# dune-community/pylrbms

Measured on AMD Instinct MI355X. Metric: offline project+estimate throughput, higher is better.
Workload: dtype f64

## Files before the change

include/lrbms_hip.h:

```cpp
#ifndef LRBMS_HIP_H
#define LRBMS_HIP_H

#include <stdint.h>

#ifdef __cplusplus
extern "C" {
#endif

#define LRBMS_OK 0
#define LRBMS_E_INVALID (-1)
#define LRBMS_E_HIP (-2)
#define LRBMS_E_STATE (-3)
#define LRBMS_E_NOT_CONVERGED (-4)

#define LRBMS_NS 16

typedef struct lrbms_ctx lrbms_ctx;

typedef struct {
  int32_t kx, ky, n_T, n_rt, n_vertices, ncf;
  double hx, hy;
  double kappa[4];
  const int32_t* nb_elem;
  const int32_t* nb_face;
// ... 52 lines not shown
} lrbms_quadrature;
int lrbms_set_quadrature(lrbms_ctx* ctx, const lrbms_quadrature* quad);

int lrbms_assemble_swipdg(lrbms_ctx* ctx, int32_t Q, const double* lam, double* A_diag, double* A_cpl, void* stream);

int lrbms_assemble_rhs(lrbms_ctx* ctx, const double* f_smp, const double* lhat, double* b, double* f2, double* ceps,
                       void* stream);

int lrbms_assemble_products(lrbms_ctx* ctx, int32_t Q, const double* theta_bar, const double* lam, const double* lam_df,
                            const double* lbar, const double* lhat, double* P_diag, double* ebar, double* caa, double* Aab,
                            double* Bbb, void* stream);

int lrbms_assemble_flux(lrbms_ctx* ctx, int32_t Q, const double* lam, double* F, void* stream);

int lrbms_oswald_apply(lrbms_ctx* ctx, int32_t N, const double* V, double* Wt, void* stream);

int lrbms_flux_reconstruct(lrbms_ctx* ctx, int32_t Q, int32_t N, const double* F, const double* V, double* Rt,
                           void* stream);

int lrbms_project_system(lrbms_ctx* ctx, int32_t Q, int32_t N, const double* V, const double* A_diag,
                         const double* A_cpl, const double* P_diag, const double* b, double* work, double* B_sys,
                         double* rhs_red, double* E_red, double* M_red, void* stream);

int64_t lrbms_estimator_work_size(lrbms_ctx* ctx, int32_t Q, int32_t N);
int lrbms_estimator_grams(lrbms_ctx* ctx, int32_t Q, int32_t N, const double* V, const double* Wt, const double* Rt,
                          const double* ebar, const double* caa, const double* Aab, const double* Bbb,
                          const double* b, double* work, double* G_nc, double* r_fd, double* G_rdd, double* G_bb,
                          double* G_ab, double* G_aa, void* stream);

int lrbms_fused_supported(lrbms_ctx* ctx, int32_t Q, int32_t N);
int32_t lrbms_fused_fnc_ld(lrbms_ctx* ctx, int32_t N);
int64_t lrbms_fused_mfma_per_subdomain(lrbms_ctx* ctx, int32_t Q, int32_t N);
int lrbms_fused_factored_supported(lrbms_ctx* ctx, int32_t Q, int32_t N);
int64_t lrbms_fused_work_size(lrbms_ctx* ctx, int32_t Q, int32_t N);
int lrbms_project_estimate_fused(lrbms_ctx* ctx, int32_t Q, int32_t N, const double* V, const double* F,
                                 const double* A_diag, const double* A_cpl, const double* P_diag, const double* b,
                                 const double* ebar, const double* caa, const double* Aab, const double* Bbb,
                                 double* work, double* B_sys, double* rhs_red, double* E_red, double* M_red,
                                 double* G_nc, double* r_fd, double* G_rdd, double* G_bb, double* G_ab, double* G_aa,
                                 void* stream);

void* lrbms_ctx_aux_stream(lrbms_ctx* ctx, int32_t i);

#define LRBMS_OPT_OSWALD_VERTEX_PATCH 9
#define LRBMS_OPT_OSWALD_ZERO_ON_SUBDOMAIN_BOUNDARY 1
#define LRBMS_OPT_ACCUMULATE_COUPLING_ACROSS_Q 2
#define LRBMS_OPT_STREAMS 3
#define LRBMS_OPT_F1_KSPLIT 4
#define LRBMS_OPT_F1_FORM 5
#define LRBMS_OPT_COARSE 6
#define LRBMS_OPT_SOLVE_VALU 7
#define LRBMS_OPT_ESTIMATE_VALU 8
#define LRBMS_OPT_PREP_LDS 10
int lrbms_ctx_set_option(lrbms_ctx* ctx, int32_t option, int32_t value);

int lrbms_set_diagonal_neighbours(lrbms_ctx* ctx, const int32_t* nbr_diag);

int lrbms_fused_set_subset(lrbms_ctx* ctx, const int32_t* subset, int32_t count);

int lrbms_kernel_timing(lrbms_ctx* ctx, int32_t enable);
int lrbms_kernel_timing_read(lrbms_ctx* ctx, char* names, int64_t names_cap, double* ms, int32_t cap, int32_t* count);

int lrbms_project_estimate_fused_phase(lrbms_ctx* ctx, int32_t phase, int32_t Q, int32_t N, const double* V, const double* F,
                                       const double* A_diag, const double* A_cpl, const double* P_diag, const double* b,
                                       const double* ebar, const double* caa, const double* Aab, const double* Bbb, double* work,
                                       double* B_sys, double* rhs_red, double* E_red, double* M_red, double* G_nc, double* r_fd,
                                       double* G_rdd, double* G_bb, double* G_ab, double* G_aa, void* stream);

int64_t lrbms_fside_size(lrbms_ctx* ctx, int32_t Q, int32_t N);
int64_t lrbms_fnc_size(lrbms_ctx* ctx, int32_t N);
int lrbms_project_estimate_fused_factored(lrbms_ctx* ctx, int32_t phase, int32_t Q, int32_t N, const double* V, const double* F,
                                          const double* A_diag, const double* A_cpl, const double* P_diag, const double* b,
                                          const double* ebar, const double* caa, const double* Aab, const double* Bbb, double* work,
                                          double* B_sys, double* rhs_red, double* E_red, double* M_red, double* G_nc_self,
                                          double* r_fd, double* G_rdd_self, double* G_bb_self, double* G_ab_self, double* G_aa,
                                          double* F_side, double* F_nc, void* stream);
int lrbms_reduced_estimate_factored(lrbms_ctx* ctx, int32_t Q, int32_t N, const double* theta, const double* u,
                                    const double* G_nc_self, const double* r_fd, const double* G_rdd_self, const double* G_bb_self,
                                    const double* G_ab_self, const double* G_aa, const double* F_side, const double* F_nc,
                                    const double* f2, const double* ceps, double hdiam, double* eta_loc, void* stream);
int lrbms_reduced_estimate_batch_factored(lrbms_ctx* ctx, int32_t Q, int32_t N, int32_t nmu, const double* theta, const double* u,
                                          const double* G_nc_self, const double* r_fd, const double* G_rdd_self,
                                          const double* G_bb_self, const double* G_ab_self, const double* G_aa, const double* F_side,
                                          const double* F_nc, const double* f2, const double* ceps, double hdiam, double* eta_loc,
                                          void* stream);

int lrbms_reduced_estimate(lrbms_ctx* ctx, int32_t Q, int32_t N, const double* theta, const double* u,
                           const double* G_nc, const double* r_fd, const double* G_rdd, const double* G_bb,
                           const double* G_ab, const double* G_aa, const double* f2, const double* ceps, double hdiam,
                           double* eta_loc, void* stream);

int lrbms_reduced_estimate_batch(lrbms_ctx* ctx, int32_t Q, int32_t N, int32_t nmu, const double* theta, const double* u,
                                 const double* G_nc, const double* r_fd, const double* G_rdd, const double* G_bb,
                                 const double* G_ab, const double* G_aa, const double* f2, const double* ceps, double hdiam,
                                 double* eta_loc, void* stream);

int64_t lrbms_reduced_solve_work_size(lrbms_ctx* ctx, int32_t N);
int lrbms_reduced_solve(lrbms_ctx* ctx, int32_t Q, int32_t N, const double* theta, const double* B_sys,
                        const double* rhs_red, double* work, double* u, double rtol, int32_t max_iter, double* info,
                        void* stream);

int64_t lrbms_reduced_solve_batch_work_size(lrbms_ctx* ctx, int32_t N, int32_t nmu);
int lrbms_reduced_solve_batch(lrbms_ctx* ctx, int32_t Q, int32_t N, int32_t nmu, const double* theta, const double* B_sys,
                              const double* rhs_red, double* work, double* u, double rtol, int32_t max_iter, double* info,
                              void* stream);

// ... 62 lines not shown
```

pylrbms_amd/_isa_check.py:

```python
import re


class IsaCheckError(RuntimeError):
    pass


def _functions(path):
    cur, out = None, {}
    with open(path) as fh:
        for ln in fh:
            m = re.match(r'^(_Z\w+):\s+; @', ln)
            if m:
                cur = m.group(1)
                out[cur] = []
                continue
            if cur is not None:
                if ln.startswith('.Lfunc_end'):
                    cur = None
                    continue
                out[cur].append(ln.rstrip('\n'))
    return out


def _metadata(path):
# ... 101 lines not shown
                break
            if op.startswith('s_cbranch') and toks and toks[-1] in label_at:
                succ.append(label_at[toks[-1]])
                continue
            touched = frozenset().union(*[_regs(t) for t in toks]) if toks else frozenset()
            if touched:
                ev.append(('T', touched, st))
        if fall and nxt[b] < len(lines):
            succ.append(nxt[b])
        blocks[b] = (ev, succ)
    bad, seen = set(), set()
    first = 0 if inside is None else max(b for b in starts if b <= min(inside))
    work = [(first, ())]
    while work:
        b, state = work.pop()
        if inside is not None and b not in inside and b != first:
            continue
        if (b, state) in seen:
            continue
        seen.add((b, state))
        if len(seen) > max_states:
            raise IsaCheckError('in-flight register analysis: more than {} (block, state) pairs'.format(max_states))
        pending = list(state)
        ev, succ = blocks[b]
        live = frozenset().union(*pending) if pending else frozenset()
        settled = False
        for e in ev:
            if e[0] == 'W':
                pending = pending[len(pending) - e[1]:] if e[1] else []
                live = frozenset().union(*pending) if pending else frozenset()
                if prologue_of is not None and not pending and b in prologue_of:
                    settled = True
                    break
            elif e[0] == 'L':
                pending = (pending + [e[1]])[-63:]
                live = live | e[1]
            elif live and e[1] & live:
                bad.add(e[2])
        if settled:
            continue
        out = tuple(pending)
        for t in succ:
            if (t, out) not in seen:
                work.append((t, out))
    return sorted(bad)


def check_fused_isa(asm_path):
    fns = _functions(asm_path)
    meta = _metadata(asm_path)
    report, problems = [], []
    seen = 0
    for name, lines in fns.items():
        m = re.search(r'\dk_f(1u|1v|1|2)I((?:Li\d+E)+)E', name) or re.search(r'\dk_f(1w)()E4Tmpl', name)
        if not m:
            continue
        kernel = 'k_f{}<{}>'.format(m.group(1), ','.join(re.findall(r'Li(\d+)E', m.group(2))))
        md = meta.get(name, {})
        spills = md.get('vgpr_spill_count', 0)
        scratch_lines = [i for i, ln in enumerate(lines) if re.match(r'\s+scratch_', ln)]
        in_asm = False
        first_asm_load = None
        for i, ln in enumerate(lines):
            st = ln.strip()
            if st.startswith(';;#ASMSTART'):
                in_asm = True
            elif st.startswith(';;#ASMEND'):
                in_asm = False
            elif in_asm and 'global_load' in ln:
                first_asm_load = i
                break
        wide = m.group(1) in ('1', '1u') and re.findall(r'Li(\d+)E', m.group(2))[0] == '4'
        if (spills or scratch_lines or md.get('private_segment_fixed_size', 0)) and not wide:
            problems.append('{}: scratch {} bytes, {} spilled VGPRs'.format(kernel, md.get('private_segment_fixed_size'), spills))
        if spills > 8:
            problems.append('{}: {} spilled VGPRs'.format(kernel, spills))
        if scratch_lines and first_asm_load is not None and max(scratch_lines) >= first_asm_load:
            problems.append('{}: scratch instruction behind the first asm-managed load (line {} >= {})'.format(
                kernel, max(scratch_lines), first_asm_load))
        lean = m.group(1) in ('1v', '1w')
        uses_asm_prefetch = any(';;#ASMSTART' in ln for ln in lines) and \
            any('global_load' in ln for ln in lines if True) and \
            any(re.search(r'^\s+s_waitcnt vmcnt\((?!0\))\d+\)\s*$' if not lean else r'^\s+s_waitcnt vmcnt\(0\)\s*$', ln) for ln in lines)
        loops, tags = _producer_loops(lines)
        if m.group(1) == '1' and kernel.endswith(',0>'):
            report.append('{}: compiler-managed loads, VGPRs {}'.format(kernel, md.get('vgpr_count')))
            continue
        if not loops or not uses_asm_prefetch:
            problems.append('{}: no producer loop with asm-managed prefetch found'.format(kernel))
            continue
        seen += 1
        if lean:
            loop_blocks = set()
            starts_all = sorted({0} | {i for i, ln in enumerate(lines) if re.match(r'^\.LBB\d+_\d+:', ln)})
            for idx in loops:
                members = set(idx)
                loop_blocks |= {b for b in starts_all if b in members}
            hz = _inflight_register_hazards(lines, tags, region=None, prologue_of=loop_blocks)
            if hz:
                problems.append('{}: compiler-emitted instruction touches the destination of an asm load of the PROLOGUE still in flight: {}'.format(
                    kernel, hz[:3]))
        for idx in loops:
            hazards = _inflight_register_hazards(lines, tags, region=idx)
            if hazards:
                problems.append('{}: compiler-emitted instruction touches the destination of an asm load still in flight: {}'.format(
                    kernel, hazards[:3]))
            a, b = idx[0], idx[-1]
# ... 45 lines not shown
```

pylrbms_amd/_native.py:

```python
import ctypes
import os

import numpy as np

_HERE = os.path.dirname(os.path.abspath(__file__))
LIB_PATH = os.path.join(_HERE, 'liblrbms_hip.so')

c_i32, c_i64, c_dbl, c_vp = ctypes.c_int32, ctypes.c_int64, ctypes.c_double, ctypes.c_void_p
_P_I32 = ctypes.POINTER(c_i32)
_P_DBL = ctypes.POINTER(c_dbl)


class MeshDesc(ctypes.Structure):
    _fields_ = ([(k, c_i32) for k in ('kx', 'ky', 'n_T', 'n_rt', 'n_vertices', 'ncf')] +
                [('hx', c_dbl), ('hy', c_dbl), ('kappa', c_dbl * 4)] +
                [(k, _P_I32) for k in ('nb_elem', 'nb_face', 'nb_elem_out', 'nb_face_out', 'elem_side_pos', 'elem_rt',
                                       'face_sign', 'dof_vertex', 'vdof_ptr', 'vdof_idx', 'rt_e0', 'rt_f0', 'rt_e1',
                                       'rt_f1', 'rt_side', 'side_elem', 'side_elem_out', 'side_count')] +
                [('ntouch', c_i32), ('touch_elem', _P_I32), ('touch_count', _P_I32)] +
                [(k, _P_DBL) for k in ('grad', 'area', 'normal', 'face_len', 'points')])


SIGNATURES = {
    'lrbms_version': (ctypes.c_char_p, []),
# ... 418 lines not shown
        self._check(rc, 'lrbms_reduced_solve')
        return u, {'iterations': int(info[0]), 'relative_residual': float(info[1])}

    def reduced_solve_batch(self, thetas, B_sys, rhs_red, rtol=1e-13, max_iter=20000, work=None):
        Q, S, N = B_sys.shape[0], self.S, B_sys.shape[3]
        th = np.ascontiguousarray(thetas, dtype=np.float64)
        nmu = th.shape[0]
        assert th.shape == (nmu, Q)
        need = int(self.lib.lrbms_reduced_solve_batch_work_size(self.handle, N, nmu))
        if work is None:
            work = self.empty(need)
        if work.numel() < need:
            raise NativeError('reduced_solve_batch: work too small')
        u = self.empty(S, N, nmu)
        info = np.zeros(2)
        rc = self.lib.lrbms_reduced_solve_batch(self.handle, Q, N, nmu, _dblp(th), self._ptr(B_sys, (Q, S, 5, N, N), 'B_sys'),
                                                self._ptr(rhs_red, (S, N), 'rhs_red'), c_vp(work.data_ptr()),
                                                c_vp(u.data_ptr()), float(rtol), int(max_iter), _dblp(info), self._stream())
        self._check(rc, 'lrbms_reduced_solve_batch')
        return u, {'iterations': int(info[0]), 'relative_residual': float(info[1])}

    def reduced_solve_batches(self, thetas, B_sys, rhs_red, per_call=64, rtol=1e-13, max_iter=20000, concat=True):
        torch = self.torch
        th = np.ascontiguousarray(thetas, dtype=np.float64)
        per_call = max(1, min(int(per_call), 64))
        work = self.empty(int(self.lib.lrbms_reduced_solve_batch_work_size(self.handle, int(B_sys.shape[3]), min(per_call, th.shape[0]))))
        res = [self.reduced_solve_batch(th[b0:b0 + per_call], B_sys, rhs_red, rtol=rtol, max_iter=max_iter, work=work)
               for b0 in range(0, th.shape[0], per_call)]
        if concat:
            u = torch.cat([r[0] for r in res], dim=2) if len(res) > 1 else res[0][0]
        else:
            u = [r[0] for r in res]
        return u, {'iterations': max(r[1]['iterations'] for r in res), 'relative_residual': max(r[1]['relative_residual'] for r in res)}

    def reduced_precond_build(self, theta, B_sys):
        Q, S, N = B_sys.shape[0], self.S, B_sys.shape[3]
        th = np.ascontiguousarray(theta, dtype=np.float64)
        assert th.shape == (Q,)
        work = self.empty(int(self.lib.lrbms_reduced_solve_work_size(self.handle, N)))
        pc = self.empty(int(self.lib.lrbms_reduced_precond_size(self.handle, N)))
        rc = self.lib.lrbms_reduced_precond_build(self.handle, Q, N, _dblp(th), self._ptr(B_sys, (Q, S, 5, N, N), 'B_sys'),
                                                  c_vp(work.data_ptr()), c_vp(pc.data_ptr()), self._stream())
        self._check(rc, 'lrbms_reduced_precond_build')
        pc._lrbms_N = N
        return pc

    def reduced_precond_use(self, pc):
        self._pc_in_use = pc
        rc = self.lib.lrbms_reduced_precond_use(self.handle, int(pc._lrbms_N) if pc is not None else 0,
                                                c_vp(pc.data_ptr()) if pc is not None else None)
        self._check(rc, 'lrbms_reduced_precond_use')

    OPTIONS = {'oswald_zero_on_subdomain_boundary': 1, 'accumulate_coupling_across_q': 2, 'oswald_vertex_patch': 9, 'prep_lds': 10,
               'streams': 3, 'f1_ksplit': 4, 'f1_form': 5, 'coarse': 6, 'solve_valu': 7, 'estimate_valu': 8}

    def set_option(self, name, value):
        if name not in self.OPTIONS:
            raise NativeError('unknown option {!r}; known: {}'.format(name, sorted(self.OPTIONS)))
        self._check(self.lib.lrbms_ctx_set_option(self.handle, self.OPTIONS[name], int(value)), 'lrbms_ctx_set_option')

    def set_diagonal_neighbours(self, nbr_diag):
        arr = np.ascontiguousarray(np.asarray(nbr_diag, dtype=np.int32))
        self._check(self.lib.lrbms_set_diagonal_neighbours(self.handle, arr.ctypes.data_as(_P_I32)), 'lrbms_set_diagonal_neighbours')

    def fused_set_subset(self, subset):
        if subset is None or len(subset) == 0:
            self._check(self.lib.lrbms_fused_set_subset(self.handle, None, 0), 'lrbms_fused_set_subset')
            return
        arr = np.ascontiguousarray(np.asarray(subset, dtype=np.int32))
        self._check(self.lib.lrbms_fused_set_subset(self.handle, arr.ctypes.data_as(_P_I32), int(arr.size)), 'lrbms_fused_set_subset')

    def fused_mfma_per_subdomain(self, Q, N):
        return int(self.lib.lrbms_fused_mfma_per_subdomain(self.handle, int(Q), int(N)))

    def kernel_timing(self, enable):
        self._check(self.lib.lrbms_kernel_timing(self.handle, 1 if enable else 0), 'lrbms_kernel_timing')

    def kernel_timing_read(self):
        cap = 256
        names = ctypes.create_string_buffer(8192)
        ms = (ctypes.c_double * cap)()
        count = c_i32(0)
        self._check(self.lib.lrbms_kernel_timing_read(self.handle, names, 8192, ms, cap, ctypes.byref(count)), 'lrbms_kernel_timing_read')
        nm = names.value.decode().split('\n') if count.value else []
        return [(nm[i], ms[i]) for i in range(count.value)]

    def aux_stream(self, i=0):
        cache = self.__dict__.setdefault('_aux_streams', {})
        if i not in cache:
            ptr = self.lib.lrbms_ctx_aux_stream(self.handle, int(i))
            if not ptr:
                raise NativeError('lrbms_ctx_aux_stream({}) returned NULL'.format(i))
            cache[i] = self.torch.cuda.ExternalStream(int(ptr), device=self.device)
        return cache[i]

    def fom_solve(self, theta, A_diag, A_cpl, b, rtol=1e-12, max_iter=100000):
        Q, S = A_diag.shape[0], self.S
        th = np.ascontiguousarray(theta, dtype=np.float64)
        assert th.shape == (Q,)
        work = self.empty(int(self.lib.lrbms_fom_solve_work_size(self.handle)))
        x = self.empty(S, self.n)
        info = np.zeros(2)
        rc = self.lib.lrbms_fom_solve(self.handle, Q, _dblp(th), self._ptr(A_diag, (Q, S, self.n_T, 4, 9), 'A_diag'),
                                      self._ptr(A_cpl, (Q, S, 4, self.ncf, 9), 'A_cpl'), self._ptr(b, (S, self.n), 'b'),
                                      c_vp(work.data_ptr()), c_vp(x.data_ptr()), float(rtol), int(max_iter), _dblp(info),
                                      self._stream())
        self._check(rc, 'lrbms_fom_solve')
# ... 219 lines not shown
```

pylrbms_amd/csrc/capi.hip:

```cpp
#include <cmath>
#include <cstring>
#include <map>
#include <mutex>

#include "lrbms_dev.h"

int64_t estimator_work_size(lrbms_ctx* ctx, int Q, int N);
int64_t reduced_solve_work_size(lrbms_ctx* ctx, int N);
int launch_reduced_estimate_batch(lrbms_ctx* ctx, int Q, int N, int nmu, const double* theta, const double* u, const double* G_nc,
                                  const double* r_fd, const double* G_rdd, const double* G_bb, const double* G_ab,
                                  const double* G_aa, const double* Fside, const double* Fnc, const double* f2, const double* ceps,
                                  double hdiam, double* eta_loc, hipStream_t st);
int64_t reduced_solve_batch_work_size(lrbms_ctx* ctx, int N, int nmu);
int launch_reduced_solve_batch(lrbms_ctx* ctx, int Q, int N, int nmu, const double* theta, const double* B_sys,
                               const double* rhs_red, double* work, double* u, double rtol, int max_iter, double* info,
                               hipStream_t st);
int launch_assemble_dcorr(lrbms_ctx* ctx, int Q, const double* lam, double* D_corr, hipStream_t st);
int64_t local_correction_work_size(lrbms_ctx* ctx, int nmark);
int launch_local_correction(lrbms_ctx* ctx, int Q, const double* theta, int nmark, const int32_t* marked, const double* A_diag,
                            const double* A_cpl, const double* D_corr, const double* b, double* work, double* corr, double rtol,
                            int max_iter, double* info, hipStream_t st);
int64_t fom_solve_work_size(lrbms_ctx* ctx);
int launch_fom_solve(lrbms_ctx* ctx, int Q, const double* theta, const double* A_diag, const double* A_cpl, const double* b,
                     double* work, double* x, double rtol, int max_iter, double* info, hipStream_t st);
// ... 114 lines not shown
  if (!ok) return lrbms_ctx_destroy(ctx), LRBMS_E_HIP;
  *out = ctx;
  return LRBMS_OK;
}

int lrbms_ctx_destroy(lrbms_ctx* ctx) {
  if (!ctx) return LRBMS_E_INVALID;
  (void)hipSetDevice(ctx->device);
  coarse_release(ctx);
  free_owned(ctx);
  if (ctx->ksp_part) (void)hipFree(ctx->ksp_part);
  if (ctx->ksp_ticket) (void)hipFree(ctx->ksp_ticket);
  if (ctx->subset) (void)hipFree(ctx->subset);
  if (ctx->wab) (void)hipFree(ctx->wab);
  for (int i = 0; i < 3; ++i) {
    if (ctx->aux[i]) lrbms_side_stream_release(ctx->device, i);
    if (ctx->ev_join[i]) (void)hipEventDestroy(ctx->ev_join[i]);
  }
  if (ctx->ev_fork) (void)hipEventDestroy(ctx->ev_fork);
  if (ctx->ev_prep) (void)hipEventDestroy(ctx->ev_prep);
  for (auto& k : ctx->ktimers) {
    if (k.e0) (void)hipEventDestroy(k.e0);
    if (k.e1) (void)hipEventDestroy(k.e1);
  }
  delete ctx;
  return LRBMS_OK;
}

void* lrbms_ctx_aux_stream(lrbms_ctx* ctx, int32_t i) { return (ctx && i >= 0 && i < 3) ? (void*)ctx->aux[i] : nullptr; }

const char* lrbms_last_error(lrbms_ctx* ctx) { return ctx ? ctx->err.c_str() : "null context"; }

int lrbms_ctx_set_option(lrbms_ctx* ctx, int32_t option, int32_t value) {
  if (!ctx) return LRBMS_E_INVALID;
  int lo = 0, hi = 1;
  if (option == LRBMS_OPT_STREAMS) lo = -1;
  if (option == LRBMS_OPT_F1_KSPLIT) hi = 4;
  if (option == LRBMS_OPT_COARSE) hi = 2;
  if (option == LRBMS_OPT_PREP_LDS) hi = 3;
  if (option == LRBMS_OPT_F1_FORM) hi = 3;
  if (value < lo || value > hi || (option == LRBMS_OPT_F1_KSPLIT && value == 3))
    return lrbms_fail(ctx, LRBMS_E_INVALID, "set_option: value out of range for this option");
  switch (option) {
    case LRBMS_OPT_OSWALD_ZERO_ON_SUBDOMAIN_BOUNDARY: ctx->t.opt_oswald_subdomain = value; break;
    case LRBMS_OPT_ACCUMULATE_COUPLING_ACROSS_Q: ctx->t.opt_accumulate_coupling = value; break;
    case LRBMS_OPT_OSWALD_VERTEX_PATCH:
      if (ctx->pass_ran && ctx->t.opt_oswald_vertex != value)
        return lrbms_fail(ctx, LRBMS_E_STATE, "set_option: LRBMS_OPT_OSWALD_VERTEX_PATCH cannot change after a fused pass has run on this context");
      ctx->t.opt_oswald_vertex = value;
      break;
    case LRBMS_OPT_STREAMS: ctx->opt_streams = value; break;
    case LRBMS_OPT_F1_KSPLIT: ctx->opt_f1_ksplit = value; break;
    case LRBMS_OPT_F1_FORM: ctx->opt_f1_legacy = value; break;
    case LRBMS_OPT_COARSE: ctx->opt_coarse = value; break;
    case LRBMS_OPT_SOLVE_VALU: ctx->opt_solve_valu = value; break;
    case LRBMS_OPT_ESTIMATE_VALU: ctx->opt_estimate_valu = value; break;
    case LRBMS_OPT_PREP_LDS: ctx->opt_prep_lds = value; break;
    default: return lrbms_fail(ctx, LRBMS_E_INVALID, "set_option: unknown option");
  }
  return LRBMS_OK;
}

int lrbms_set_diagonal_neighbours(lrbms_ctx* ctx, const int32_t* nbr_diag) {
  LRBMS_REQUIRE_MESH(ctx);
  if (!nbr_diag) return lrbms_fail(ctx, LRBMS_E_INVALID, "set_diagonal_neighbours: null table");
  for (long i = 0; i < (long)ctx->S * 4; ++i)
    if (nbr_diag[i] < -1 || nbr_diag[i] >= ctx->S_ext)
      return lrbms_fail(ctx, LRBMS_E_INVALID, "set_diagonal_neighbours: index out of range [-1, S_ext)");
  LRBMS_HIP_CHECK(ctx, hipDeviceSynchronize());
  LRBMS_HIP_CHECK(ctx, hipMemcpy(const_cast<int*>(ctx->t.nbr_diag), nbr_diag, sizeof(int) * (size_t)ctx->S * 4, hipMemcpyHostToDevice));
  ctx->diag_explicit = true;
  return LRBMS_OK;
}

int lrbms_fused_set_subset(lrbms_ctx* ctx, const int32_t* subset, int32_t count) {
  LRBMS_REQUIRE_MESH(ctx);
  if (count < 0 || count > ctx->S || (count > 0 && subset == nullptr))
    return lrbms_fail(ctx, LRBMS_E_INVALID, "fused_set_subset: count must be in [0, S] and the list non-null");
  for (int i = 0; i < count; ++i)
    if (subset[i] < 0 || subset[i] >= ctx->S || (i > 0 && subset[i] <= subset[i - 1]))
      return lrbms_fail(ctx, LRBMS_E_INVALID, "fused_set_subset: the list must be strictly ascending local subdomain indices in [0, S)");
  if (count > ctx->subset_cap) {
    if (ctx->subset) LRBMS_HIP_CHECK(ctx, hipFree(ctx->subset));
    ctx->subset = nullptr;
    ctx->subset_cap = 0;
    LRBMS_HIP_CHECK(ctx, hipMalloc(&ctx->subset, sizeof(int) * (size_t)ctx->S));
    ctx->subset_cap = ctx->S;
  }
  if (count > 0) {
    LRBMS_HIP_CHECK(ctx, hipDeviceSynchronize());
    LRBMS_HIP_CHECK(ctx, hipMemcpy(ctx->subset, subset, sizeof(int) * (size_t)count, hipMemcpyHostToDevice));
  }
  ctx->subset_n = count;
  return LRBMS_OK;
}

int lrbms_kernel_timing(lrbms_ctx* ctx, int32_t enable) {
  if (!ctx) return LRBMS_E_INVALID;
  ctx->ktime = enable != 0;
  ctx->ktime_n = 0;
  for (auto& k : ctx->ktimers) k.used = false;
  return LRBMS_OK;
}

int lrbms_kernel_timing_read(lrbms_ctx* ctx, char* names, int64_t names_cap, double* ms, int32_t cap, int32_t* count) {
  if (!ctx || !names || !ms || !count || names_cap <= 0) return LRBMS_E_INVALID;
// ... 530 lines not shown
```

pylrbms_amd/csrc/fused.hip:

```cpp
#include <cstdlib>
#include <map>
#include <mutex>
#include <type_traits>

#include "lrbms_dev.h"

namespace {

typedef double d4 __attribute__((ext_vector_type(4)));
typedef double d2 __attribute__((ext_vector_type(2)));
template <int W> struct VecT { using T = double; };
template <> struct VecT<2> { using T = d2; };
template <int W> __device__ inline typename VecT<W>::T ldv(const double* p) { return *reinterpret_cast<const typename VecT<W>::T*>(p); }
template <int W> __device__ inline void stv(double* p, typename VecT<W>::T v) { *reinterpret_cast<typename VecT<W>::T*>(p) = v; }
template <int W> __device__ inline typename VecT<W>::T zerov() { return typename VecT<W>::T(0.0); }
using W1 = std::integral_constant<int, 1>;
using W2 = std::integral_constant<int, 2>;

#if !defined(LRBMS_EXPERIMENT_BUILD) &&                                                                               \
    (defined(F1_NO_STAGE) || defined(F1_NO_APPLY) || defined(F1_NO_VALU_STAGE) || defined(F1_NO_MFMA) ||             \
     defined(F1_LDS_FILL) || defined(F1_PRODUCER_PRIO) || defined(F1_SPLIT_SIMD) || defined(F1_PF) ||                \
     defined(F2_NO_STAGE) || defined(F2_NO_MFMA) || defined(F1_TRACE) || defined(F1V_NO_STORE) || defined(F1V_NO_MIRROR) || defined(F3_EW_X) || defined(PREP_TRACE) || defined(THIN_TRACE))
#error "experiment switch defined in a product build of fused.hip (use tools/build_variant.sh, which sets LRBMS_EXPERIMENT_BUILD)"
#endif
#ifndef F1_SPLIT_SIMD
#define F1_SPLIT_SIMD 0
#endif
#ifndef F1_PF
#define F1_PF 1
#endif
#ifdef F1_TRACE
__device__ unsigned long long g_f1_trace[2][64][8];
#define F1_STAMP(role, c, k)                                                                                   \
  do {                                                                                                         \
    if (blockIdx.x == 0 && blockIdx.y == 0 && blockIdx.z == 0 && (threadIdx.x & 63) == 0 && (c) < 64)        \
      g_f1_trace[role][c][k] = __builtin_amdgcn_s_memtime();                                                  \
  } while (0)
extern "C" int lrbms_debug_f1_trace(unsigned long long* host) {
  return (int)hipMemcpyFromSymbol(host, HIP_SYMBOL(g_f1_trace), sizeof(g_f1_trace));
}
#else
#define F1_STAMP(role, c, k) do {} while (0)
#endif
#ifdef THIN_TRACE
__device__ unsigned long long g_thin_trace[3][8];
#define THIN_STAMP(z, k)                                                                                       \
  do {                                                                                                         \
    if (side == 1 && s == 500 && threadIdx.x == 0) g_thin_trace[z][k] = __builtin_amdgcn_s_memtime();          \
  } while (0)
extern "C" int lrbms_debug_thin_trace(unsigned long long* host) {
  return (int)hipMemcpyFromSymbol(host, HIP_SYMBOL(g_thin_trace), sizeof(g_thin_trace));
}
#else
#define THIN_STAMP(z, k) do {} while (0)
#endif
#ifdef PREP_TRACE
__device__ unsigned long long g_prep_trace[2][16];
#define PREP_STAMP(k)                                                                                          \
  do {                                                                                                         \
    if (blockIdx.x == 5 && prep_trace_on && (threadIdx.x == 0 || threadIdx.x == PREP_LDS_THREADS - 64))        \
      g_prep_trace[threadIdx.x == 0 ? 0 : 1][k] = __builtin_amdgcn_s_memtime();                               \
  } while (0)
extern "C" int lrbms_debug_prep_trace(unsigned long long* host) {
  return (int)hipMemcpyFromSymbol(host, HIP_SYMBOL(g_prep_trace), sizeof(g_prep_trace));
}
#else
#define PREP_STAMP(k) do {} while (0)
#endif
constexpr int EC = 4;
constexpr int F1_NTY = 7;
constexpr int F1_MAXG = 12;

__host__ __device__ constexpr int padded_ld(int tiles) { return (tiles * 16) % 32 == 16 ? tiles * 16 : tiles * 16 + 16; }

__device__ inline int uniform(int x) { return __builtin_amdgcn_readfirstlane(x); }

typedef const __attribute__((address_space(4))) int* cint_p;
typedef const __attribute__((address_space(4))) double* cdbl_p;

// ... 2605 lines not shown
      int idx = ((cw + s) & (NCW - 1)) + k * NCW, i = 0;
      if (idx >= NTRI) idx = -1;
      int rem = idx;
      while (rem >= NR - i && idx >= 0) {
        rem -= NR - i;
        ++i;
      }
      ti[k] = idx >= 0 ? i : -1;
      tj[k] = idx >= 0 ? i + rem : 0;
    }
    d4 accb[TPW], accd[TPW];
#pragma unroll
    for (int k = 0; k < TPW; ++k) accb[k] = accd[k] = (d4){0.0, 0.0, 0.0, 0.0};
    for (int c = 0; c < nchunks; ++c) {
      lds_barrier();
      const double* xb = &Xb[c & 1][0];
      const double* yb = &Yb[c & 1][0];
      const double* xd = &Xd[c & 1][0];
      const double* yd = &Yd[c & 1][0];
#pragma unroll
      for (int k = 0; k < TPW; ++k) {
        if (ti[k] < 0) continue;
        const int xo = ti[k] * 16 + li, yo = tj[k] * 16 + li;
#ifndef F2_NO_MFMA
#pragma unroll
        for (int kk = 0; kk < 3 * EC; kk += 4)
          accb[k] = __builtin_amdgcn_mfma_f64_16x16x4f64(xb[(kk + lk) * LD + xo], yb[(kk + lk) * LD + yo], accb[k], 0, 0, 0);
        accd[k] = __builtin_amdgcn_mfma_f64_16x16x4f64(xd[lk * LD + xo], yd[lk * LD + yo], accd[k], 0, 0, 0);
#else
        (void)xb; (void)yb; (void)xd; (void)yd; (void)xo; (void)yo;
#endif
      }
    }
    lds_barrier();
    double* gb = a.G_bb + (long)s * a.gstride;
    double* gd = a.G_rdd + (long)s * a.gstride;
#pragma unroll
    for (int k = 0; k < TPW; ++k) {
      if (ti[k] < 0) continue;
      const int col = tj[k] * 16 + li;
#pragma unroll
      for (int r = 0; r < 4; ++r) {
        const int row = ti[k] * 16 + lk + 4 * r;
        const double vb = accb[k][r], vd = accd[k][r];
        if (col < QN && row < QN) {
          gb[(long)row * QN + col] = vb;
          gd[(long)row * QN + col] = vd;
          if (ti[k] != tj[k]) {
            gb[(long)col * QN + row] = vb;
            gd[(long)col * QN + row] = vd;
          }
        }
      }
    }
  }
  __syncthreads();
  for (int c = tid; c < QN; c += nthreads) {
    double sum = 0.0;
    for (int w = 0; w < EC; ++w) sum += red[w * 128 + c];
    a.r_fd[(long)s * C + 2 * QN + c] = sum;
  }
}

struct F3Args {
  const double *V, *ebar, *AvgSelf, *AvgSide;
  double* G_nc;
  int N, S;
  long gsub;
  int gld, goff;
};

#ifndef F3_EW_X
#define F3_EW_X 4
#endif
constexpr int F3_EW = F3_EW_X;

template <int NTX>
__global__ __launch_bounds__(256) void k_f3(Tmpl t, F3Args a) {
  constexpr int LD = padded_ld(NTX);
  constexpr int ECH = 4 * F3_EW;
  constexpr int NTRI = NTX * (NTX + 1) / 2;
  constexpr int NT = (NTRI + 3) / 4;
  __shared__ double Xs[3 * ECH * LD], Ys[3 * ECH * LD];
  const int s = subdomain_of(t, blockIdx.x), tid = threadIdx.x, lane = tid & 63, li = lane & 15, lk = lane >> 4;
  const int wave = uniform(tid >> 6);
  const int N = a.N;
  for (int i = tid; i < 3 * ECH * LD; i += 256) Xs[i] = Ys[i] = 0.0;
  int ti[NT], tj[NT];
#pragma unroll
  for (int k = 0; k < NT; ++k) {
    int idx = wave + 4 * k, i = 0;
    if (idx >= NTRI) idx = -1;
    int rem = idx;
    while (idx >= 0 && rem >= NTX - i) {
      rem -= NTX - i;
      ++i;
    }
    ti[k] = idx >= 0 ? i : -1;
    tj[k] = idx >= 0 ? i + rem : 0;
  }
  __syncthreads();
  d4 acc[NT];
#pragma unroll
  for (int i = 0; i < NT; ++i) acc[i] = (d4){0.0, 0.0, 0.0, 0.0};
  const double* Vs = a.V + (long)s * t.n * N;
  const double* As = a.AvgSelf + (long)s * t.nv * N;
// ... 1427 lines not shown
      hipLaunchKernelGGL(k_thin_expand, dim3(4, Sg), dim3(256), lds3, s_rt, t, e);
      LRBMS_LAUNCH_CHECK(ctx);
    }
  }
  if (do_b && !merge_thin) {
    hipStream_t side = s_nc;
    if (phase != 0 && !side_from_lds) {
      KScope ks(ctx, "k_vertex_side", side);
      hipLaunchKernelGGL(k_vertex_side, dim3(grid_for((long)Sg * 4 * nvs * N)), dim3(256), 0, side, t, S, ctx->nbr, N, V, AvgSide);
    }
    const int ntx = (N + 15) / 16;
    if (factored) {
      const ThinNcfArgs f{V, ebar, AvgSelf, AvgSide, ctx->nbr, Fnc, N, S};
      const size_t ldsf = thin_ncf_lds_bytes(t, N);
      if (ldsf > 64 * 1024)
        LRBMS_HIP_CHECK(ctx, hipFuncSetAttribute((const void*)k_thin_ncf, hipFuncAttributeMaxDynamicSharedMemorySize, (int)ldsf));
      KScope ks(ctx, "k_thin_ncf", side);
      hipLaunchKernelGGL(k_thin_ncf, dim3(4, Sg), dim3(256), ldsf, side, t, f);
    } else {
    const size_t lds = thin_nc_lds_bytes(t, ntx);
#define LRBMS_THIN_NC(NTX)                                                                                                       \
  do {                                                                                                                           \
    if (lds > 64 * 1024)                                                                                                         \
      LRBMS_HIP_CHECK(ctx, hipFuncSetAttribute((const void*)k_thin_nc<NTX>, hipFuncAttributeMaxDynamicSharedMemorySize, (int)lds)); \
    hipLaunchKernelGGL(k_thin_nc<NTX>, dim3(4, Sg), dim3(512), lds, side, t, S, ctx->nbr, N, V, ebar, AvgSelf, AvgSide, G_nc);    \
  } while (0)
    {
    KScope ks(ctx, "k_thin_nc", side);
    switch (ntx) {
      case 1: LRBMS_THIN_NC(1); break;
      case 2: LRBMS_THIN_NC(2); break;
      case 3: LRBMS_THIN_NC(3); break;
      default: LRBMS_THIN_NC(4); break;
    }
    }
#undef LRBMS_THIN_NC
    }
    LRBMS_LAUNCH_CHECK(ctx);
    ThinRtArgs a{V, Rself, Rside, Bbb, Aab, b, ctx->nbr, Fside, r_fd, Q, N, S};
    const size_t lds2 = thin_rt_lds_bytes(t, Q, N);
    {
      KScope ks(ctx, "k_thin_rt", s_rt);
      hipLaunchKernelGGL(k_thin_rt, dim3(4, Sg), dim3(256), lds2, s_rt, t, a);
    }
    LRBMS_LAUNCH_CHECK(ctx);
    if (!factored) {
      ThinExpandArgs e{Fside, ctx->nbr, G_bb, G_rdd, G_ab, Q, N, S};
      const size_t lds3 = sizeof(double) * (size_t)t.ncf * fside_ld(Q, N);
      KScope ks(ctx, "k_thin_expand", s_rt);
      hipLaunchKernelGGL(k_thin_expand, dim3(4, Sg), dim3(256), lds3, s_rt, t, e);
      LRBMS_LAUNCH_CHECK(ctx);
    }
  }
  if (do_a) {
    F2Args a{Rself, Bbb, b, ctx->nbr, G_bb, G_rdd, r_fd, Q, N, S, gstride};
    const int nr = (QN + 15) / 16;
    const size_t ldsf2 = sizeof(double) * 4 * t.nT + sizeof(int) * 3 * t.nT;
#define LRBMS_F2(NRV)                                                                                                       \
  do {                                                                                                                       \
    if (ldsf2 > 64 * 1024)                                                                                                   \
      LRBMS_HIP_CHECK(ctx, hipFuncSetAttribute((const void*)k_f2<NRV>, hipFuncAttributeMaxDynamicSharedMemorySize, (int)ldsf2)); \
    hipLaunchKernelGGL(k_f2<NRV>, dim3(Sg), dim3(64 * (F2_NCW + EC)), ldsf2, s_f23, t, a);                                    \
  } while (0)
    KScope ks(ctx, "k_f2", s_f23);
    switch (nr) {
      case 1: LRBMS_F2(1); break;
      case 2: LRBMS_F2(2); break;
      case 3: LRBMS_F2(3); break;
      case 4: LRBMS_F2(4); break;
      case 5: LRBMS_F2(5); break;
      case 6: LRBMS_F2(6); break;
      case 7: LRBMS_F2(7); break;
      default: LRBMS_F2(8); break;
    }
#undef LRBMS_F2
    LRBMS_LAUNCH_CHECK(ctx);
  }
  if (do_a && !(prep_from_lds && gnc_fold)) {
    F3Args a{V, ebar, AvgSelf, AvgSide, G_nc, N, S, factored ? (long)N * N : 25L * N * N, factored ? N : 5 * N,
             factored ? 0 : 10 * N * N + 2 * N};
    const int ntx = (N + 15) / 16;
    KScope ks(ctx, "k_f3", s_f3);
    switch (ntx) {
      case 1: hipLaunchKernelGGL(k_f3<1>, dim3(Sg), dim3(256), 0, s_f3, t, a); break;
      case 2: hipLaunchKernelGGL(k_f3<2>, dim3(Sg), dim3(256), 0, s_f3, t, a); break;
      case 3: hipLaunchKernelGGL(k_f3<3>, dim3(Sg), dim3(256), 0, s_f3, t, a); break;
      default: hipLaunchKernelGGL(k_f3<4>, dim3(Sg), dim3(256), 0, s_f3, t, a); break;
    }
    LRBMS_LAUNCH_CHECK(ctx);
  }
  if (do_b && !merge_thin) {
    const int ntx = (N + 15) / 16;
    const size_t ldsc = coupling_lds_bytes(t, ntx, Q);
    KScope ks(ctx, "k_coupling", s_rt);
#define LRBMS_CPL(NTXV)                                                                                                      \
  do {                                                                                                                       \
    if (ldsc > 64 * 1024)                                                                                                    \
      LRBMS_HIP_CHECK(ctx, hipFuncSetAttribute((const void*)k_coupling<NTXV>, hipFuncAttributeMaxDynamicSharedMemorySize, (int)ldsc)); \
    hipLaunchKernelGGL(k_coupling<NTXV>, dim3(4, Sg), dim3(256), ldsc, s_rt, t, S, ctx->nbr, Q, N, V, A_cpl, B_sys);          \
  } while (0)
    switch (ntx) {
      case 1: LRBMS_CPL(1); break;
      case 2: LRBMS_CPL(2); break;
      case 3: LRBMS_CPL(3); break;
      default: LRBMS_CPL(4); break;
    }
#undef LRBMS_CPL
    LRBMS_LAUNCH_CHECK(ctx);
  }
// ... 8 lines not shown
```

pylrbms_amd/csrc/lrbms_dev.h:

```cpp
#pragma once
#include <hip/hip_runtime.h>
#include <stdint.h>
#include <string>
#include <vector>

#include "../../include/lrbms_hip.h"

struct Tmpl {
  int kx, ky, nT, n, nrt, nv, nvx, nvy, ncf;
  double hx, hy;
  double kappa[4], kinv[4], kmin;
  const int *nb_elem, *nb_face, *nb_elem_out, *nb_face_out, *elem_side_pos, *elem_rt, *face_sign;
  const int *dof_vertex, *vdof_ptr, *vdof_idx;
  const int *rt_e0, *rt_f0, *rt_e1, *rt_f1, *rt_side;
  const int *side_elem, *side_elem_out, *side_count;
  int ntouch;
  const int *touch_elem, *touch_count;
  const double *grad, *area, *normal, *face_len, *points;
  const double* stiff;
  const double* mass9;
  const double* zero64;
  const double* lgz;
  const double* hab;
  const int* touch_vtx;
  const int* touch_pos;
  const int* touch_mask;
  const int* touch_rlist;
  const int* sface_i;
  const double* sface_d;
  int opt_oswald_subdomain;
  int opt_oswald_vertex;
  int opt_accumulate_coupling;
  const int* sub_list;
  int sub_count;
  const int* nbr_diag;
};

__device__ inline int subdomain_of(const Tmpl& t, int b) { return t.sub_list ? t.sub_list[b] : b; }

hipStream_t lrbms_side_stream_acquire(int device, int i);
void lrbms_side_stream_release(int device, int i);

struct lrbms_ctx {
  int device = 0;
  int num_cus = 0;
  bool has_mesh = false;
  Tmpl t{};
  int S = 0, S_ext = 0;
  int* nbr = nullptr;
  std::vector<int32_t> nbr_host;
  std::vector<void*> owned;
  hipStream_t aux[3] = {nullptr, nullptr, nullptr};
  hipEvent_t ev_fork = nullptr, ev_join[3] = {nullptr, nullptr, nullptr};
  hipEvent_t ev_prep = nullptr;
  hipEvent_t prep_done = nullptr;
  void* blas = nullptr;
  double* coarse = nullptr;
  long coarse_cap = 0;
  bool ktime = false;
  struct KTimer { const char* name; hipEvent_t e0, e1; bool used; };
  std::vector<KTimer> ktimers;
  int ktime_n = 0;
  double* ksp_part = nullptr;
  long ksp_part_cap = 0;
  int* ksp_ticket = nullptr;
  long ksp_ticket_cap = 0;
  double* wab = nullptr;
  long wab_cap = 0;
  const double* wab_src = nullptr;
  int wab_Q = 0;
  bool pass_ran = false;
  bool diag_explicit = false;
  int* subset = nullptr;
  int subset_n = 0, subset_cap = 0;
  lrbms_quadrature* qdev = nullptr;
  int opt_streams = -1, opt_f1_ksplit = 0, opt_f1_legacy = 0, opt_coarse = 1, opt_solve_valu = 0, opt_estimate_valu = 0, opt_prep_lds = 1;
  const double* user_pc = nullptr;
  int user_pc_N = 0;
  std::string err;
};

#define SIGMA_INNER 8.0
#define SIGMA_BOUNDARY 14.0

__host__ __device__ inline int side_to_slot(int side) { return side < 2 ? side : side + 1; }
__host__ __device__ inline int slot_to_side(int slot) { return slot < 2 ? slot : slot - 1; }

static inline int lrbms_fail(lrbms_ctx* ctx, int code, const std::string& msg) {
  if (ctx) ctx->err = msg;
  return code;
}

#define LRBMS_HIP_CHECK(ctx, expr)                                                                  \
  do {                                                                                              \
    hipError_t _e = (expr);                                                                         \
    if (_e != hipSuccess)                                                                           \
      return lrbms_fail(ctx, LRBMS_E_HIP, std::string(#expr) + ": " + hipGetErrorString(_e));       \
  } while (0)

#define LRBMS_REQUIRE_MESH(ctx)                                                      \
  do {                                                                               \
    if (!(ctx)) return LRBMS_E_INVALID;                                              \
    if (!(ctx)->has_mesh) return lrbms_fail(ctx, LRBMS_E_STATE, "mesh not uploaded"); \
  } while (0)

#define LRBMS_LAUNCH_CHECK(ctx) LRBMS_HIP_CHECK(ctx, hipGetLastError())

struct KScope {
  lrbms_ctx* ctx;
  hipStream_t st;
  int idx;
  KScope(lrbms_ctx* c, const char* name, hipStream_t s) : ctx(c), st(s), idx(-1) {
    if (!c->ktime) return;
    if (c->ktime_n == (int)c->ktimers.size()) {
      lrbms_ctx::KTimer k{name, nullptr, nullptr, false};
      if (hipEventCreate(&k.e0) != hipSuccess || hipEventCreate(&k.e1) != hipSuccess) return;
      c->ktimers.push_back(k);
    }
    idx = c->ktime_n++;
    c->ktimers[idx].name = name;
    c->ktimers[idx].used = true;
    (void)hipEventRecord(c->ktimers[idx].e0, st);
  }
  ~KScope() {
    if (idx >= 0) (void)hipEventRecord(ctx->ktimers[idx].e1, st);
  }
};

int build_template_tables(lrbms_ctx* ctx);
// ... 33 lines not shown
```

Baseline: 1.504 million.

## Add Cholesky-factored Gram form of f2 estimator kernel with triangle-tile wave plan

Adds a new k_f2g kernel, on by default when LDS fits, that factors each element's 3x3 Bbb block by Cholesky. Producer waves stage the factored residual rows and face-divergence rows into double-buffered LDS. Consumer waves then form the G_bb and G_rdd Gram blocks with f64 MFMA over upper-triangle tiles only, mirroring the off-diagonal results and using a constexpr greedy plan that splits tiles across waves while sharing fragments. The aim is to cut redundant MFMA work and the per-element matrix application of the previous f2 form. The cost is more LDS per block, per-element square roots, NaN output for non-SPD blocks, and more kernel instantiations.

```diff
diff --git a/include/lrbms_hip.h b/include/lrbms_hip.h
--- a/include/lrbms_hip.h
+++ b/include/lrbms_hip.h
@@ -128,6 +128,7 @@
 #define LRBMS_OPT_SOLVE_VALU 7
 #define LRBMS_OPT_ESTIMATE_VALU 8
 #define LRBMS_OPT_PREP_LDS 10
+#define LRBMS_OPT_F2_FORM 11
 int lrbms_ctx_set_option(lrbms_ctx* ctx, int32_t option, int32_t value);
 
 int lrbms_set_diagonal_neighbours(lrbms_ctx* ctx, const int32_t* nbr_diag);
diff --git a/pylrbms_amd/_isa_check.py b/pylrbms_amd/_isa_check.py
--- a/pylrbms_amd/_isa_check.py
+++ b/pylrbms_amd/_isa_check.py
@@ -177,7 +177,7 @@
     report, problems = [], []
     seen = 0
     for name, lines in fns.items():
-        m = re.search(r'\dk_f(1u|1v|1|2)I((?:Li\d+E)+)E', name) or re.search(r'\dk_f(1w)()E4Tmpl', name)
+        m = re.search(r'\dk_f(1u|1v|1|2g|2)I((?:Li\d+E)+)E', name) or re.search(r'\dk_f(1w)()E4Tmpl', name)
         if not m:
             continue
         kernel = 'k_f{}<{}>'.format(m.group(1), ','.join(re.findall(r'Li(\d+)E', m.group(2))))
diff --git a/pylrbms_amd/_native.py b/pylrbms_amd/_native.py
--- a/pylrbms_amd/_native.py
+++ b/pylrbms_amd/_native.py
@@ -494,7 +494,8 @@
         self._check(rc, 'lrbms_reduced_precond_use')
 
     OPTIONS = {'oswald_zero_on_subdomain_boundary': 1, 'accumulate_coupling_across_q': 2, 'oswald_vertex_patch': 9, 'prep_lds': 10,
-               'streams': 3, 'f1_ksplit': 4, 'f1_form': 5, 'coarse': 6, 'solve_valu': 7, 'estimate_valu': 8}
+               'streams': 3, 'f1_ksplit': 4, 'f1_form': 5, 'coarse': 6, 'solve_valu': 7, 'estimate_valu': 8,
+               'f2_form': 11}
 
     def set_option(self, name, value):
         if name not in self.OPTIONS:
diff --git a/pylrbms_amd/csrc/capi.hip b/pylrbms_amd/csrc/capi.hip
--- a/pylrbms_amd/csrc/capi.hip
+++ b/pylrbms_amd/csrc/capi.hip
@@ -190,6 +190,7 @@
     case LRBMS_OPT_STREAMS: ctx->opt_streams = value; break;
     case LRBMS_OPT_F1_KSPLIT: ctx->opt_f1_ksplit = value; break;
     case LRBMS_OPT_F1_FORM: ctx->opt_f1_legacy = value; break;
+    case LRBMS_OPT_F2_FORM: ctx->opt_f2_form = value; break;
     case LRBMS_OPT_COARSE: ctx->opt_coarse = value; break;
     case LRBMS_OPT_SOLVE_VALU: ctx->opt_solve_valu = value; break;
     case LRBMS_OPT_ESTIMATE_VALU: ctx->opt_estimate_valu = value; break;
diff --git a/pylrbms_amd/csrc/fused.hip b/pylrbms_amd/csrc/fused.hip
--- a/pylrbms_amd/csrc/fused.hip
+++ b/pylrbms_amd/csrc/fused.hip
@@ -2,6 +2,7 @@
 #include <map>
 #include <mutex>
 #include <type_traits>
+#include <utility>
 
 #include "lrbms_dev.h"
 
@@ -20,11 +21,14 @@
 #if !defined(LRBMS_EXPERIMENT_BUILD) &&                                                                               \
     (defined(F1_NO_STAGE) || defined(F1_NO_APPLY) || defined(F1_NO_VALU_STAGE) || defined(F1_NO_MFMA) ||             \
      defined(F1_LDS_FILL) || defined(F1_PRODUCER_PRIO) || defined(F1_SPLIT_SIMD) || defined(F1_PF) ||                \
-     defined(F2_NO_STAGE) || defined(F2_NO_MFMA) || defined(F1_TRACE) || defined(F1V_NO_STORE) || defined(F1V_NO_MIRROR) || defined(F3_EW_X) || defined(PREP_TRACE) || defined(THIN_TRACE))
+     defined(F2_NO_STAGE) || defined(F2_NO_MFMA) || defined(F2G_WG) || defined(F1_TRACE) || defined(F1V_NO_STORE) || defined(F1V_NO_MIRROR) || defined(F3_EW_X) || defined(PREP_TRACE) || defined(THIN_TRACE))
 #error "experiment switch defined in a product build of fused.hip (use tools/build_variant.sh, which sets LRBMS_EXPERIMENT_BUILD)"
 #endif
 #ifndef F1_SPLIT_SIMD
 #define F1_SPLIT_SIMD 0
+#endif
+#ifndef F2G_WG
+#define F2G_WG 3
 #endif
 #ifndef F1_PF
 #define F1_PF 1
@@ -2736,6 +2740,223 @@
           }
         }
       }
+    }
+  }
+  __syncthreads();
+  for (int c = tid; c < QN; c += nthreads) {
+    double sum = 0.0;
+    for (int w = 0; w < EC; ++w) sum += red[w * 128 + c];
+    a.r_fd[(long)s * C + 2 * QN + c] = sum;
+  }
+}
+
+constexpr int F2G_ROWS = 4 * EC;
+constexpr int F2G_EL = 8;
+
+template <int NR>
+struct F2gPlan {
+  static constexpr int NTRI = NR * (NR + 1) / 2, NCW = F2_NCW, TPW = (NTRI + NCW - 1) / NCW;
+  int nt[NCW] = {}, nf[NCW] = {};
+  int frag[NCW][NR] = {};
+  int ta[NCW][TPW] = {}, tb[NCW][TPW] = {};
+  constexpr F2gPlan() {
+    bool used[NTRI] = {};
+    for (int w = 0; w < NCW; ++w) {
+      const int want = NTRI / NCW + (w < NTRI % NCW ? 1 : 0);
+      int local[NR] = {};
+      for (int i = 0; i < NR; ++i) local[i] = -1;
+      for (int k = 0; k < want; ++k) {
+        int best = -1, bi = 0, bj = 0, bcost = 3;
+        for (int i = 0, idx = 0; i < NR; ++i)
+          for (int j = i; j < NR; ++j, ++idx) {
+            if (used[idx]) continue;
+            const int cost = (local[i] < 0 ? 1 : 0) + (j != i && local[j] < 0 ? 1 : 0);
+            if (cost < bcost) { bcost = cost; best = idx; bi = i; bj = j; }
+          }
+        used[best] = true;
+        if (local[bi] < 0) { local[bi] = nf[w]; frag[w][nf[w]++] = bi; }
+        if (local[bj] < 0) { local[bj] = nf[w]; frag[w][nf[w]++] = bj; }
+        ta[w][k] = local[bi];
+        tb[w][k] = local[bj];
+        ++nt[w];
+      }
+    }
+  }
+};
+
+template <int... I, class F>
+__device__ inline void static_for(std::integer_sequence<int, I...>, F&& f) {
+  (f(std::integral_constant<int, I>{}), ...);
+}
+
+template <int NR, int ROLE>
+__device__ inline void f2g_consume(const double* buf, int nchunks, double* gb, double* gd, int QN, int li, int lk) {
+  constexpr int LD = padded_ld(NR);
+  constexpr F2gPlan<NR> P{};
+  constexpr int NT = P.nt[ROLE], NF = P.nf[ROLE];
+  if constexpr (NT == 0) {
+    for (int c = 0; c <= nchunks; ++c) lds_barrier();
+  } else {
+    d4 accb[NT], accd[NT];
+#pragma unroll
+    for (int k = 0; k < NT; ++k) accb[k] = accd[k] = (d4){0.0, 0.0, 0.0, 0.0};
+    for (int c = 0; c < nchunks; ++c) {
+      lds_barrier();
+      const double* x = buf + (c & 1) * F2G_ROWS * LD + lk * LD + li;
+#pragma unroll
+      for (int ks = 0; ks < 4; ++ks) {
+        double f[NF];
+        static_for(std::make_integer_sequence<int, NF>{}, [&](auto u) { f[u] = x[4 * ks * LD + P.frag[ROLE][u] * 16]; });
+#ifndef F2_NO_MFMA
+        static_for(std::make_integer_sequence<int, NT>{}, [&](auto k) {
+          constexpr int A = P.ta[ROLE][k], B = P.tb[ROLE][k];
+          if (ks < 3) accb[k] = __builtin_amdgcn_mfma_f64_16x16x4f64(f[A], f[B], accb[k], 0, 0, 0);
+          else accd[k] = __builtin_amdgcn_mfma_f64_16x16x4f64(f[A], f[B], accd[k], 0, 0, 0);
+        });
+#else
+        (void)f;
+#endif
+      }
+    }
+    lds_barrier();
+    static_for(std::make_integer_sequence<int, NT>{}, [&](auto k) {
+      constexpr int TI = P.frag[ROLE][P.ta[ROLE][k]], TJ = P.frag[ROLE][P.tb[ROLE][k]];
+      const int col = TJ * 16 + li;
+#pragma unroll
+      for (int r = 0; r < 4; ++r) {
+        const int row = TI * 16 + lk + 4 * r;
+        const double vb = accb[k][r], vd = accd[k][r];
+        if (col < QN && row < QN) {
+          gb[(long)row * QN + col] = vb;
+          gd[(long)row * QN + col] = vd;
+          if (TI != TJ) {
+            gb[(long)col * QN + row] = vb;
+            gd[(long)col * QN + row] = vd;
+          }
+        }
+      }
+    });
+  }
+}
+
+inline size_t f2g_dyn_lds_bytes(const Tmpl& t) { return sizeof(double) * (F2G_EL + 4) * (size_t)t.nT + sizeof(int) * 3 * (size_t)t.nT; }
+template <int NR>
+constexpr size_t f2g_static_lds_bytes() { return sizeof(double) * (2 * F2G_ROWS * padded_ld(NR) + EC * 128); }
+
+template <int NR>
+__global__ __launch_bounds__(64 * (F2_NCW + EC)) __attribute__((amdgpu_waves_per_eu(NR <= 5 ? 2 * F2G_WG : 2))) void k_f2g(Tmpl t, F2Args a) {
+  constexpr int LD = padded_ld(NR);
+  extern __shared__ double dyn[];
+  __shared__ double Xg[2 * F2G_ROWS * LD];
+  __shared__ double red[EC * 128];
+  const int s = subdomain_of(t, blockIdx.x), tid = threadIdx.x, lane = tid & 63, li = lane & 15, lk = lane >> 4;
+  const int wave = uniform(tid >> 6);
+  const int nthreads = 64 * (F2_NCW + EC);
+  const int QN = a.Q * a.N, C = 5 * QN;
+  double* fac = dyn;
+  double* coefs = dyn + F2G_EL * t.nT;
+  double* bsums = coefs + 3 * t.nT;
+  int* rts = reinterpret_cast<int*>(bsums + t.nT);
+  const int* nbr_s = a.nbr + s * 5;
+  for (int i = tid; i < 3 * t.nT; i += nthreads) {
+    const int T = i / 3, f = i - 3 * T;
+    coefs[i] = face_sign_at(t, nbr_s, T, f) * t.face_len[i] / t.area[T];
+    rts[i] = t.elem_rt[i];
+  }
+  for (int T = tid; T < t.nT; T += nthreads) {
+    const double* be = a.b + (long)s * t.n + 3 * T;
+    bsums[T] = be[0] + be[1] + be[2];
+    const double* B = a.Bbb + ((long)s * t.nT + T) * 9;
+    const double p0 = B[0];
+    const double c00 = sqrt(p0), c01 = B[1] / c00, c02 = B[2] / c00;
+    const double p1 = B[4] - c01 * c01;
+    const double c11 = sqrt(p1), c12 = (B[5] - c01 * c02) / c11;
+    const double p2 = B[8] - c02 * c02 - c12 * c12;
+    const double c22 = sqrt(p2);
+    const bool spd = p0 > 0.0 && p1 > 0.0 && p2 > 0.0;
+    const double nan = __builtin_nan("");
+    double* ft = fac + F2G_EL * T;
+    ft[0] = spd ? c00 : nan;
+    ft[1] = spd ? c01 : nan;
+    ft[2] = spd ? c02 : nan;
+    ft[3] = spd ? c11 : nan;
+    ft[4] = spd ? c12 : nan;
+    ft[5] = spd ? c22 : nan;
+    ft[6] = sqrt(t.area[T]);
+    ft[7] = 0.0;
+  }
+  for (int i = tid; i < 2 * F2G_ROWS * LD; i += nthreads) Xg[i] = 0.0;
+  for (int i = tid; i < EC * 128; i += nthreads) red[i] = 0.0;
+  __syncthreads();
+  const int nchunks = t.nT / EC;
+  const double* Rs = a.Rself + (long)s * t.nrt * QN;
+
+  if (wave < EC) {
+    double rv[2][3], nrv[2][3];
+    const int cc0 = lane < QN ? lane : QN - 1, cc1 = lane + 64 < QN ? lane + 64 : QN - 1;
+    auto load = [&](int T, double (&r)[2][3]) {
+      const int r0 = rts[3 * T], r1 = rts[3 * T + 1], r2 = rts[3 * T + 2];
+      r[0][0] = gload_f64(Rs + (long)r0 * QN + cc0);
+      r[0][1] = gload_f64(Rs + (long)r1 * QN + cc0);
+      r[0][2] = gload_f64(Rs + (long)r2 * QN + cc0);
+      r[1][0] = gload_f64(Rs + (long)r0 * QN + cc1);
+      r[1][1] = gload_f64(Rs + (long)r1 * QN + cc1);
+      r[1][2] = gload_f64(Rs + (long)r2 * QN + cc1);
+    };
+    auto wait_set = [&](double (&r)[2][3]) {
+      asm volatile("s_waitcnt vmcnt(6)" : "+v"(r[0][0]), "+v"(r[0][1]), "+v"(r[0][2]), "+v"(r[1][0]), "+v"(r[1][1]), "+v"(r[1][2]));
+    };
+    auto wait_set_tie = [&](double (&r)[2][3]) {
+      asm volatile("" : "+v"(r[0][0]), "+v"(r[0][1]), "+v"(r[0][2]), "+v"(r[1][0]), "+v"(r[1][1]), "+v"(r[1][2]));
+    };
+    load(wave, rv);
+    double rfd_part[2] = {0.0, 0.0};
+    auto step = [&](int c, double (&cr)[2][3], double (&nr)[2][3]) {
+      const int T = c * EC + wave, el = wave;
+      load(c + 1 < nchunks ? T + EC : T, nr);
+      wait_set(cr);
+      double* xb = Xg + (c & 1) * F2G_ROWS * LD;
+      const double* ft = fac + F2G_EL * T;
+      const double u00 = ft[0], u01 = ft[1], u02 = ft[2], u11 = ft[3], u12 = ft[4], u22 = ft[5], sqa = ft[6];
+      const double c0f = coefs[3 * T], c1f = coefs[3 * T + 1], c2f = coefs[3 * T + 2];
+      const double bsum = bsums[T];
+#pragma unroll
+      for (int k = 0; k < 2; ++k) {
+        const int cc = lane + 64 * k;
+#ifdef F2_NO_STAGE
+        if (cc < QN && cr[k][0] == 1.2345e300) {
+#else
+        if (cc < QN) {
+#endif
+          const double rv0 = cr[k][0], rv1 = cr[k][1], rv2 = cr[k][2];
+          xb[(3 * el) * LD + cc] = u00 * rv0 + u01 * rv1 + u02 * rv2;
+          xb[(3 * el + 1) * LD + cc] = u11 * rv1 + u12 * rv2;
+          xb[(3 * el + 2) * LD + cc] = u22 * rv2;
+          const double d = c0f * rv0 + c1f * rv1 + c2f * rv2;
+          xb[(3 * EC + el) * LD + cc] = sqa * d;
+          rfd_part[k] += bsum * d;
+        }
+      }
+      lds_barrier();
+    };
+    for (int c = 0; c < nchunks; c += 2) {
+      step(c, rv, nrv);
+      step(c + 1, nrv, rv);
+    }
+    lds_barrier();
+    asm volatile("s_waitcnt vmcnt(0)" ::: "memory");
+    wait_set_tie(rv);
+    wait_set_tie(nrv);
+    red[wave * 128 + lane] = rfd_part[0];
+    red[wave * 128 + 64 + lane] = rfd_part[1];
+  } else {
+    double* gb = a.G_bb + (long)s * a.gstride;
+    double* gd = a.G_rdd + (long)s * a.gstride;
+    switch ((wave - EC + s) & (F2_NCW - 1)) {
+      case 0: f2g_consume<NR, 0>(Xg, nchunks, gb, gd, QN, li, lk); break;
+      case 1: f2g_consume<NR, 1>(Xg, nchunks, gb, gd, QN, li, lk); break;
+      case 2: f2g_consume<NR, 2>(Xg, nchunks, gb, gd, QN, li, lk); break;
+      default: f2g_consume<NR, 3>(Xg, nchunks, gb, gd, QN, li, lk); break;
     }
   }
   __syncthreads();
@@ -4269,9 +4490,35 @@
       LRBMS_LAUNCH_CHECK(ctx);
     }
   }
-  if (do_a) {
+  const int nr2 = (QN + 15) / 16;
+  static const size_t f2g_static[8] = {f2g_static_lds_bytes<1>(), f2g_static_lds_bytes<2>(), f2g_static_lds_bytes<3>(), f2g_static_lds_bytes<4>(),
+                                       f2g_static_lds_bytes<5>(), f2g_static_lds_bytes<6>(), f2g_static_lds_bytes<7>(), f2g_static_lds_bytes<8>()};
+  const bool f2_gram = ctx->opt_f2_form == 0 && f2g_dyn_lds_bytes(t) + f2g_static[nr2 - 1] <= 160 * 1024;
+  if (do_a && f2_gram) {
     F2Args a{Rself, Bbb, b, ctx->nbr, G_bb, G_rdd, r_fd, Q, N, S, gstride};
-    const int nr = (QN + 15) / 16;
+    const size_t ldsf2 = f2g_dyn_lds_bytes(t);
+#define LRBMS_F2G(NRV)                                                                                                      \
+  do {                                                                                                                       \
+    LRBMS_HIP_CHECK(ctx, raise_max_lds(ctx->device, (const void*)k_f2g<NRV>, (int)ldsf2));                                  \
+    hipLaunchKernelGGL(k_f2g<NRV>, dim3(Sg), dim3(64 * (F2_NCW + EC)), ldsf2, s_f23, t, a);                                   \
+  } while (0)
+    KScope ks(ctx, "k_f2", s_f23);
+    switch (nr2) {
+      case 1: LRBMS_F2G(1); break;
+      case 2: LRBMS_F2G(2); break;
+      case 3: LRBMS_F2G(3); break;
+      case 4: LRBMS_F2G(4); break;
+      case 5: LRBMS_F2G(5); break;
+      case 6: LRBMS_F2G(6); break;
+      case 7: LRBMS_F2G(7); break;
+      default: LRBMS_F2G(8); break;
+    }
+#undef LRBMS_F2G
+    LRBMS_LAUNCH_CHECK(ctx);
+  }
+  if (do_a && !f2_gram) {
+    F2Args a{Rself, Bbb, b, ctx->nbr, G_bb, G_rdd, r_fd, Q, N, S, gstride};
+    const int nr = nr2;
     const size_t ldsf2 = sizeof(double) * 4 * t.nT + sizeof(int) * 3 * t.nT;
 #define LRBMS_F2(NRV)                                                                                                       \
   do {                                                                                                                       \
diff --git a/pylrbms_amd/csrc/lrbms_dev.h b/pylrbms_amd/csrc/lrbms_dev.h
--- a/pylrbms_amd/csrc/lrbms_dev.h
+++ b/pylrbms_amd/csrc/lrbms_dev.h
@@ -74,7 +74,7 @@
   int* subset = nullptr;
   int subset_n = 0, subset_cap = 0;
   lrbms_quadrature* qdev = nullptr;
-  int opt_streams = -1, opt_f1_ksplit = 0, opt_f1_legacy = 0, opt_coarse = 1, opt_solve_valu = 0, opt_estimate_valu = 0, opt_prep_lds = 1;
+  int opt_streams = -1, opt_f1_ksplit = 0, opt_f1_legacy = 0, opt_coarse = 1, opt_solve_valu = 0, opt_estimate_valu = 0, opt_prep_lds = 1, opt_f2_form = 0;
   const double* user_pc = nullptr;
   int user_pc_N = 0;
   std::string err;
```

Result: faster. 1.531 million (median of 6 runs) (+1.8%).
